# ArchieGertsman/gym-sparksched

Measured on AMD Instinct MI355X. Metric: scheduling decisions/sec (env steps/s), higher is better.
Workload: dtype f64+i32

## Files before the change

gym-sparksched_amd/csrc/decima_rollout.h:

```cpp
#pragma once
#include <type_traits>

#include "kernels.h"
#include "decima.h"
#include "decima_policy.h"

#ifndef SSIM_DR_EX_LDS
#define SSIM_DR_EX_LDS 0
#endif

struct DecimaWork {
  int64_t feat_scratch, plan, stride;
  int64_t feats, ccap, emask, depth;
  int64_t packed, total;
};
inline DecimaWork decima_work(const ssim_layout& L) {
  DecimaWork w{};
  w.feat_scratch = 0;
  w.plan = align16(decima_scratch_bytes(L.stage_cap));
  w.stride = (w.plan + decima_policy_lds_bytes(L.stage_cap, L.job_cap) + 255) & ~int64_t(255);
  int64_t o = w.stride * L.num_envs;
  w.feats = o;
  o = align16(o + (int64_t)L.num_envs * L.stage_cap * kDecimaFeatures * 4);
  w.ccap = o;
// ... 23 lines not shown
template <bool kHelp = false, bool kGreedy = false>
__device__ __forceinline__ DpAction decima_decide(
    const Params* P0, const uint8_t* obs0, const dp_f32x4* weights0, uint8_t* feat_scratch0, uint8_t* plan0,
    float* feats0, int32_t* ccap0, uint32_t* emask0, int32_t* depth0, float num_tasks_scale, float work_scale,
    uint64_t seed, uint64_t ctr, int eid, int plan_cap, uint32_t plan_lds, uint64_t* pprof, uint32_t help_lds = 0) {
  using W = WaveHip;
  const Params* P = (const Params*)(const SSIM_GLOBAL Params*)P0;
  const uint8_t* obs = (const uint8_t*)(const SSIM_GLOBAL uint8_t*)obs0;
  const dp_f32x4* weights = (const dp_f32x4*)(const SSIM_GLOBAL dp_f32x4*)weights0;
  float* feats = (float*)(SSIM_GLOBAL float*)feats0;
  int32_t* ccap = (int32_t*)(SSIM_GLOBAL int32_t*)ccap0;
  uint32_t* emask = (uint32_t*)(SSIM_GLOBAL uint32_t*)emask0;
  int32_t* depth = (int32_t*)(SSIM_GLOBAL int32_t*)depth0;
  const ssim_layout& L = P->L;
  const DecimaPolicyOut none{nullptr, nullptr, nullptr, nullptr, nullptr, nullptr, nullptr};
  const DpWGlobal wts{weights};
  DpAction act;
  DpHelp* const help = kHelp ? reinterpret_cast<DpHelp*>(g_smem + help_lds) : nullptr;
#ifdef SSIM_PROFILE
  uint64_t tp = W::clock();
#endif
#ifdef SSIM_DR_GLOBAL_ONLY
  if (false) {
#else
  if (plan_cap > 0) {
#endif
    uint8_t* pl = g_smem + plan_lds;
    DecimaView<W>{L, obs, eid}.template run<false>(num_tasks_scale, work_scale, pl, feats, ccap, emask, depth,
                                                   plan_cap);
#ifdef SSIM_PROFILE
    if (pprof != nullptr && W::lane() == 0) W::lds_add_u64(pprof - kPhDecParts + kPhDecFeat, W::clock() - tp);
#endif
    decima_policy_env<false, kHelp, kGreedy>(P, obs, feats, ccap, emask, depth, wts, plan_cap, seed, ctr, eid, pl, none, &act,
                                    pprof, kDpLdsDags, help);
  } else {
    uint8_t* fs = (uint8_t*)(SSIM_GLOBAL uint8_t*)feat_scratch0;
    uint8_t* pg = (uint8_t*)(SSIM_GLOBAL uint8_t*)plan0;
    DecimaView<W>{L, obs, eid}.template run<true>(num_tasks_scale, work_scale, fs, feats, ccap, emask, depth);
#ifdef SSIM_PROFILE
    if (pprof != nullptr && W::lane() == 0) W::lds_add_u64(pprof - kPhDecParts + kPhDecFeat, W::clock() - tp);
#endif
    decima_policy_env<true, kHelp, kGreedy>(P, obs, feats, ccap, emask, depth, wts, L.stage_cap, seed, ctr, eid, pg, none, &act,
                                   pprof, 0, help);
  }
  return act;
}

struct DecimaTimedNone {};
template <bool kTimed>
using DecimaTimedArgs = std::conditional_t<kTimed, ssim_decima_timed, DecimaTimedNone>;
template <bool kHelp = false, bool kTimed = false, bool kGreedy = false>
struct DecimaPolicy {
  static constexpr bool kTimedMode = kTimed;
  const Params* P;
  const uint8_t* obs;
  DecimaRolloutArgs a;
  DecimaTimedArgs<kTimed> t;

  template <class S>
  __device__ __forceinline__ bool in_time(const S& s) const {
    if constexpr (kTimed) return WaveHip::uni(t.clock[2 * (int64_t)s.eid]) < t.duration;
    return true;
  }
  template <class S>
  __device__ __forceinline__ bool next_episode(const S& s) const {
    if constexpr (kTimed) {
      using W = WaveHip;
      int32_t* sc = t.sched + 2 * (int64_t)s.eid;
      if (W::uni(sc[0]) < t.cap_resets) return true;
      W::sync();
      if (W::lane() == 0) sc[1] = 1;
      W::sync();
      return false;
    }
    return true;
  }
  template <class S>
  __device__ __forceinline__ void reset_episode(S& s, uint8_t* rec) const {
    if constexpr (kTimed) {
      using W = WaveHip;
      const int eid = s.eid;
      int32_t* sc = t.sched + 2 * (int64_t)eid;
      const int64_t slot = (int64_t)eid * t.cap_resets + W::uni(sc[0]);
      const uint64_t seed = W::uni(t.seeds[slot]);
      const double limit = W::uni(t.limits[slot]);
      const int last = W::uni(a.smp.cursor[(int64_t)eid * 8]) - 1;
      const int J = s.JC;
      for (int j = W::lane(); j < J; j += W::kWidth) {
        t.ep_arrival[slot * J + j] = s.jtimes(j).tarr;
        t.ep_completed[slot * J + j] = s.jtimes(j).tdone;
        t.ep_state[slot * J + j] = s.job(j).state;
      }
      W::sync();
      if (W::lane() == 0) {
        t.reset_steps[slot] = last;
        sc[0] = sc[0] + 1;
      }
      W::sync();
      s.reset_sampled(SSIM_RESET_SEED, seed, limit, rec);
    }
  }

  template <class S>
  __device__ __forceinline__ bool can_act(const S& s) const {
    using W = WaveHip;
    if (!a.autoreset && (s.h.terminated || s.frozen() || s.h.wall >= s.h.time_limit || s.h.num_jobs == 0))
// ... 261 lines not shown
```

gym-sparksched_amd/csrc/engine.h:

```cpp
#pragma once
#include <stddef.h>
#include <stdint.h>

#include "layout.h"
#include "pcg64.h"
#include "pyset.h"

#ifdef SSIM_PROFILE
#define SSIM_TIC(v) const uint64_t v = W::clock()
#define SSIM_TOC(v, ph) prof_add(ph, W::clock() - (v))
#else
#define SSIM_TIC(v) (void)0
#define SSIM_TOC(v, ph) (void)0
#endif

#ifdef SSIM_MARKERS
#define SSIM_MARK(name) asm volatile("; SSIM_MARK " name)
#else
#define SSIM_MARK(name) (void)0
#endif

#if defined(__clang__)
#pragma clang fp contract(off)
#endif

namespace ssim {

template <class W, class = void>
struct KatBadPage {
  static constexpr bool value = false;
};
template <class W>
struct KatBadPage<W, decltype((void)W::kKatBadPage)> {
  static constexpr bool value = W::kKatBadPage;
};

#if defined(__HIP_DEVICE_COMPILE__)
#define SSIM_GLOBAL __attribute__((address_space(1)))
#else
#define SSIM_GLOBAL
#endif
template <class T>
__device__ __forceinline__ T ldg(const T* p, int64_t i) {
  return ((const SSIM_GLOBAL T*)p)[i];
}

enum : int32_t { kPhPolicy = 0, kPhAction, kPhRoundCheck, kPhFulfill, kPhPop, kPhHandle, kPhPostScan, kPhObserve,
                 kPhSample, kPhPool, kPhScan, kPhLoadSave, kPhPoolBig, kPhIdleOrder, kPhDraw, kPhJobArr,
                 kPhExecArr, kPhTaskDone, kPhStageDone,
                 kPhIter,
                 kCtPoolSmall, kCtPoolBig, kCtTask, kCtIdleOrder,
                 kHist0,
                 kTEntry = kHist0 + 16, kTLoaded, kTLoopEnd, kTSaved, kTCtor, kTCopy1,
                 kPhDecFeat, kPhDecPolicy, kPhDecRecord,
                 kPhDecParts,
                 kPhReset = kPhDecParts + 10, kCtReset,
                 kCtNoEvent, kCtPredPass, kCtDeltaObs, kNumPhases };
static_assert(kNumPhases <= 64, "StateOffsets::sc_prof holds 64 sums");
#ifdef SSIM_PROFILE
#define SSIM_COUNT(ph) prof_add(ph, 1)
#else
#define SSIM_COUNT(ph) (void)0
#endif
#ifndef SSIM_POOL_STAT
#define SSIM_POOL_STAT(op, size, used) (void)0
#endif
#ifndef SSIM_FIELD_STAT
#define SSIM_FIELD_STAT(sec) (void)0
#endif
enum : int32_t { kPoolNone = -1, kPoolCommon = 0 };
enum : int32_t { kEvArrival = 1, kEvTask = 2, kEvReady = 3, kTrJobDone = 4, kTrToCommon = 5 };
enum : int32_t { kJobPending = 0, kJobActive = 1, kJobDone = 2 };
enum : int32_t { kScanAll = 0, kScanOnly = 1, kScanExcept = 2 };

struct StepIn {
  int32_t stage_idx, num_exec;
};

struct NoStop {
  static constexpr bool kCan = false;
  __device__ __forceinline__ uint64_t issue() const { return 0; }
  __device__ __forceinline__ bool hit(uint64_t) const { return false; }
};
enum : int32_t { kSimIdle = 0, kSimDecision = 1, kSimPreempted = 2 };

struct HotParams {
  const int32_t* tpl_stage_base;
  const int32_t* ts_num_tasks;
  const double* ts_rough;
  const int32_t* ts_child_base;
  const int32_t* ts_children;
  const int32_t* ts_parent_base;
  const int32_t* ts_parents;
  const int32_t* ts_fw_keymask;
  const int32_t* ts_fw_maxlevel;
  const int32_t* dur_off;
  const int32_t* dur_len;
  const double* durations;
  const uint64_t* ts_topo;
  double moving_delay, warmup_delay, beta, job_arrival_gap;
  int64_t ob_nodes, ob_edge_links, ob_dag_ptr, ob_supplies, ob_frontier, ob_sched_rank, ob_counts, ob_reward,
      ob_wall_time, ob_acc, ob_trace;
  int32_t num_templates, trace_cap, edge_cap, job_arrival_cap, topo;
  int32_t dcache;
};
static_assert(sizeof(HotParams) <= 256 && sizeof(HotParams) % 8 == 0, "one dword per lane of one VGPR");

constexpr int kIvRows = 256;
struct Params {
  HotParams hp;
  ssim_layout L;
// ... 18 lines not shown
  memset(p->iv, 0, sizeof(p->iv));
  for (int n = 0; n <= num_executors && n < kIvRows; ++n) {
    const double lo = intervals[2 * n], hi = intervals[2 * n + 1];
    if (!(lo >= 0 && lo <= 255 && hi >= 0 && hi <= 255 && lo == (double)(int)lo && hi == (double)(int)hi))
      return false;
    p->iv[n][0] = (uint8_t)lo;
    p->iv[n][1] = (uint8_t)hi;
    p->iv[n][2] = (uint8_t)exec_level_index(lo);
    p->iv[n][3] = (uint8_t)exec_level_index(hi);
  }
  return true;
}

inline void fill_hot_params(Params* p) {
  HotParams& h = p->hp;
  const ssim_dataset& D = p->D;
  h.tpl_stage_base = D.tpl_stage_base;
  h.ts_num_tasks = D.ts_num_tasks;
  h.ts_rough = D.ts_rough;
  h.ts_child_base = D.ts_child_base;
  h.ts_children = D.ts_children;
  h.ts_parent_base = D.ts_parent_base;
  h.ts_parents = D.ts_parents;
  h.ts_fw_keymask = D.ts_fw_keymask;
  h.ts_fw_maxlevel = D.ts_fw_maxlevel;
  h.dur_off = D.dur_off;
  h.dur_len = D.dur_len;
  h.durations = D.durations;
  h.ts_topo = D.ts_topo;
  h.moving_delay = p->C.moving_delay;
  h.warmup_delay = p->C.warmup_delay;
  h.beta = p->C.beta;
  h.job_arrival_gap = p->C.job_arrival_gap;
  const ssim_layout& L = p->L;
  h.ob_nodes = L.ob_nodes;
  h.ob_edge_links = L.ob_edge_links;
  h.ob_dag_ptr = L.ob_dag_ptr;
  h.ob_supplies = L.ob_supplies;
  h.ob_frontier = L.ob_frontier;
  h.ob_sched_rank = L.ob_sched_rank;
  h.ob_counts = L.ob_counts;
  h.ob_reward = L.ob_reward;
  h.ob_wall_time = L.ob_wall_time;
  h.ob_acc = L.ob_acc;
  h.ob_trace = L.ob_trace;
  h.num_templates = D.num_templates;
  h.trace_cap = L.trace_cap;
  h.edge_cap = L.edge_cap;
  h.job_arrival_cap = p->C.job_arrival_cap;
  h.topo = (p->C.max_stages <= 32 && D.ts_topo != nullptr) ? 1 : 0;
  h.dcache = 0;
}

template <class W, int kN = 0, int kJ = 0, int kS = 0>
struct Sim {
  using WT = W;
  const ssim_layout& L;
  const ssim_dataset& D;
  const ssim_config& C;
  const uint8_t (*IV)[4];
  const int32_t NE, JC, SC;
  const StateOffsets O;
  uint8_t* ghot;
  uint8_t* hot;
  uint8_t* cold;
  uint8_t* scr;
  uint8_t* obs;
  int32_t eid;
  bool res;
  bool row_lds;
  bool ex_l;
  uint8_t* xb;
  EnvHeader h;
  Pcg64 rng;
  uint32_t iv_lane;
#ifndef SSIM_EV_PAGES_GENERIC
#define SSIM_EV_PAGES_GENERIC 1
#endif
#ifndef SSIM_DUR_CACHE
#define SSIM_DUR_CACHE 1
#endif
  static constexpr int kEvPages = W::kWidth == 64 ? (kN > 0 ? (kN + 63) / 64 : SSIM_EV_PAGES_GENERIC) : 0;
  struct EvRegs {
    uint32_t tlo, thi;
    int32_t seq;
    int32_t ts;
  };
  EvRegs evr[kEvPages > 0 ? kEvPages : 1];
  __device__ __forceinline__ bool ev_in_regs() const { return kEvPages > 0 && NE <= 64 * kEvPages; }
  static constexpr bool kDurCache = W::kWidth == 64 && kN > 0 && kN <= kDurCacheMaxExecs && SSIM_DUR_CACHE;
  bool dcache_on = false;
  __device__ __forceinline__ bool dc_on() const { return kDurCache && dcache_on; }
  const HotParams* HPp;
  uint32_t hpv;
#ifdef SSIM_PROFILE
  uint64_t* prof;
  __device__ __forceinline__ void prof_add(int ph, uint64_t v) {
    if (W::lane() == 0) W::lds_add_u64(prof + ph, v);
  }
  __device__ __forceinline__ void prof_set(int ph, uint64_t v) {
    W::sync();
    if (W::lane() == 0) prof[ph] = v;
    W::sync();
  }
#endif

  __device__ __forceinline__ Sim(const Params* __restrict__ p, uint8_t* state_arena, uint8_t* lds,
                                 uint8_t* obs_arena, int32_t env_index, bool resident, bool row_cold = false,
                                 bool ex_lds = false)
// ... 221 lines not shown
    __device__ __forceinline__ UF& operator-=(int v) {
      SSIM_FIELD_STAT(kSec);
      *p = (T)(*p - v);
      return *this;
    }
  };
  template <class T>
  __device__ __forceinline__ T ld(const T* q) const {
    return W::uni(*q);
  }
  template <class T>
  __device__ __forceinline__ T ldu(const T* q, int64_t i) const {
    return W::uni(ldg(q, i));
  }

  template <class R>
  __device__ __forceinline__ R ld_rec(const R& src) const {
    static_assert(sizeof(R) % 4 == 0, "records are whole words");
    uint32_t w[sizeof(R) / 4];
    __builtin_memcpy(w, &src, sizeof(R));
    for (int i = 0; i < (int)(sizeof(R) / 4); ++i) w[i] = W::uni(w[i]);
    R r;
    __builtin_memcpy(&r, w, sizeof(R));
    return r;
  }

  __device__ __forceinline__ StageRec& stage(int g) const { return H<StageRec>(O.stages)[g]; }
  __device__ __forceinline__ JobRec& job(int j) const { return H<JobRec>(O.jobs)[j]; }
  __device__ __forceinline__ JobTimes& jtimes(int j) const { return H<JobTimes>(O.jtimes)[j]; }
  __device__ __forceinline__ ExecRec& exr(int e) const { return reinterpret_cast<ExecRec*>(xb)[e]; }
  __device__ __forceinline__ CommitRec& cm(int k) const { return H<CommitRec>(O.commits)[k]; }
  __device__ __forceinline__ PoolRec& pool(int p) const { return H<PoolRec>(O.pools)[p]; }
  __device__ __forceinline__ double* recent() const { return reinterpret_cast<double*>(cold + O.st_recent); }
  __device__ __forceinline__ UF<int16_t, 0> st_job(int g) const { return {&stage(g).job}; }
  __device__ __forceinline__ UF<int16_t, 0> st_ts(int g) const { return {&stage(g).ts}; }
  __device__ __forceinline__ UF<int16_t, 0> st_rem(int g) const { return {&stage(g).rem}; }
  __device__ __forceinline__ UF<int16_t, 0> st_exe(int g) const { return {&stage(g).exe}; }
  __device__ __forceinline__ UF<int16_t, 0> st_mov(int g) const { return {&stage(g).mov}; }
  __device__ __forceinline__ UF<int16_t, 0> st_com(int g) const { return {&stage(g).com}; }
  __device__ __forceinline__ UF<int8_t, 0> st_unmet(int g) const { return {&stage(g).unmet}; }
  __device__ __forceinline__ UF<uint8_t, 0> st_sel(int g) const { return {&stage(g).sel}; }
  __device__ __forceinline__ UF<double, 6> st_recent(int g) const { return {recent() + g}; }
  __device__ __forceinline__ bool st_completed(int g) const { return st_rem(g) == 0 && st_exe(g) == 0; }
  __device__ __forceinline__ UF<int16_t, 1> job_tpl(int j) const { return {&job(j).tpl}; }
  __device__ __forceinline__ UF<int16_t, 1> job_base(int j) const { return {&job(j).base}; }
  __device__ __forceinline__ UF<int16_t, 1> job_nst(int j) const { return {&job(j).nst}; }
  __device__ __forceinline__ UF<int16_t, 1> job_nact(int j) const { return {&job(j).nact}; }
  __device__ __forceinline__ UF<int16_t, 1> job_sat(int j) const { return {&job(j).sat}; }
  __device__ __forceinline__ UF<int16_t, 1> job_local(int j) const { return {&job(j).local}; }
  __device__ __forceinline__ UF<int16_t, 1> job_supply(int j) const { return {&job(j).supply}; }
  __device__ __forceinline__ UF<int16_t, 1> job_state(int j) const { return {&job(j).state}; }
  __device__ __forceinline__ UF<int32_t, 1> job_arr_dec(int j) const { return {&job(j).arr_dec}; }
  __device__ __forceinline__ UF<int32_t, 1> job_done_dec(int j) const { return {&job(j).done_dec}; }
  __device__ __forceinline__ UF<double, 2> job_tarr(int j) const { return {&jtimes(j).tarr}; }
  __device__ __forceinline__ UF<double, 2> job_tdone(int j) const { return {&jtimes(j).tdone}; }
  __device__ __forceinline__ UF<int16_t, 3> ex_loc(int e) const { return {&exr(e).loc}; }
  __device__ __forceinline__ UF<int16_t, 3> ex_job(int e) const { return {&exr(e).job}; }
  __device__ __forceinline__ UF<int16_t, 3> ex_task(int e) const { return {&exr(e).task}; }
  __device__ __forceinline__ UF<int16_t, 3> ex_busy(int e) const { return {&exr(e).busy}; }
  __device__ __forceinline__ UF<double, 4> ev_t(int e) const { return {&exr(e).ev_t}; }
  __device__ __forceinline__ UF<int32_t, 4> ev_seq(int e) const { return {&exr(e).ev_seq}; }
  __device__ __forceinline__ UF<int16_t, 4> ev_type(int e) const { return {&exr(e).ev_type}; }
  __device__ __forceinline__ UF<int16_t, 4> ev_stage(int e) const { return {&exr(e).ev_stage}; }
  __device__ __forceinline__ int32_t job_pool(int j) const { return 1 + j; }
  __device__ __forceinline__ int32_t stage_pool(int g) const { return 1 + JC + g; }
  __device__ __forceinline__ bool is_stage_pool(int p) const { return p > JC; }
  __device__ __forceinline__ int32_t pool_stage(int p) const { return p - 1 - JC; }
  __device__ __forceinline__ int32_t pool_job(int p) const {
    if (p <= 0) return -1;
    if (p <= JC) return p - 1;
    return st_job(p - 1 - JC);
  }
  __device__ __forceinline__ PySetMeta* pmeta(int p) const { return reinterpret_cast<PySetMeta*>(&pool(p)); }
  __device__ __forceinline__ uint8_t* ptab(int p) const { return cold + O.pool_tab + (int64_t)p * tab_stride_for(NE); }
  __device__ __forceinline__ UF<int16_t, 5> cfrom(int p) const { return {&pool(p).cfrom}; }
  __device__ __forceinline__ int pool_size(int p) const { return p < 0 ? 0 : (int)W::uni(pool(p).used); }

  __device__ __forceinline__ int32_t source_job() const {
    return (h.source <= kPoolCommon) ? -1 : pool_job(h.source);
  }
  __device__ __forceinline__ int committable() {
    if (h.source < 0) return 0;
    SSIM_FIELD_STAT(10);
    const PoolRec pr = pool(h.source);
    const int n = (int)W::uni(pr.used) - (int)W::uni(pr.cfrom);
    check(n >= 0);
    return n;
  }
  __device__ __forceinline__ int demand(int g) const { return st_rem(g) - (st_mov(g) + st_com(g)); }

  __device__ __forceinline__ void supply_add(int job, int n) {
    if (job < 0)
      h.supply_none += n;
    else
      job_supply(job) += n;
  }

  __device__ __forceinline__ void add_commitment(int n, int dst) {
    const int src = h.source;
    check(src >= 0);
    if (src < 0) return;
    int hit = -1, freeslot = -1;
    SSIM_FIELD_STAT(13);
    const int hw = h.commit_hw;
    for (int k0 = 0; k0 < commit_cap_for(NE); k0 += W::kWidth) {
      if (k0 >= hw) break;
// ... 1177 lines not shown
      release_idle_one(src, e);
      return;
    }
    goto_stage(e, pool_stage(dst));
  }

  __device__ __forceinline__ void fulfill_from_source() {
    int32_t* idle = S<int32_t>(O.sc_keys_a);
    int32_t* plan = S<int32_t>(O.sc_plan);
    const int n_idle = idle_order(h.source, idle);
    const int n_plan = h.source >= 0 ? commit_plan(h.source, plan) : 0;
    int k = 0;
    for (int c = 0; c < n_plan; ++c) {
      const int dst = ld(plan + 2 * c);
      int n = ld(plan + 2 * c + 1);
      check(dst >= 0 && n > 0);
      while (n > 0 && k < n_idle && !frozen()) {
        const int e = ld(idle + k++);
        fulfill(e, dst);
        n--;
      }
    }
    check(k == n_idle);
  }

  __device__ __forceinline__ void commit_leftovers() {
    const int n = committable();
    if (n > 0) add_commitment(n, kPoolCommon);
  }

  __device__ __forceinline__ bool release(int e, int g, bool changed) {
    const int dst = peek_commitment(stage_pool(g));
    if (dst != kPoolNone) {
      fulfill(e, dst);
      return true;
    }
    ex_task(e) = -1;
    if (changed) release_idle_one(stage_pool(g), e);
    return false;
  }

  __device__ __forceinline__ void on_job_arrival(int j) {
    job_state(j) = kJobActive;
    job_arr_dec(j) = h.decisions;
    int16_t* aj = H<int16_t>(O.active_jobs);
    int16_t* as = H<int16_t>(O.active_stages);
    if (W::lane() == 0) aj[h.n_active_jobs] = (int16_t)j;
    const int base = job_base(j), n = job_nst(j), tsb = ldu(HP(tpl_stage_base), (int)job_tpl(j));
    const int32_t* const nt = HP(ts_num_tasks);
    const int32_t* const pb = HP(ts_parent_base);
    const int32_t* const fwk = HP(ts_fw_keymask);
    const int32_t* const fwm = HP(ts_fw_maxlevel);
    const double* const rough = HP(ts_rough);
    for (int k0 = 0; k0 <= n; k0 += W::kWidth) {
      const int k = k0 + W::lane();
      if (k <= n) {
        const int p = (k == n) ? job_pool(j) : stage_pool(base + k);
        ps_init(pmeta(p), pool(p).tab);
        cfrom(p) = 0;
        if (k < n) {
          const int g = base + k, ts = tsb + k;
          StageRec r;
          r.job = (int16_t)j;
          r.ts = (int16_t)ts;
          r.rem = (int16_t)ldg(nt, ts);
          r.exe = 0;
          r.mov = 0;
          r.com = 0;
          r.unmet = (int8_t)(ldg(pb, ts + 1) - ldg(pb, ts));
          r.sel = 0;
          r.fw_keymask = (uint8_t)ldg(fwk, ts);
          r.fw_maxlevel = (uint8_t)ldg(fwm, ts);
          stage(g) = r;
          recent()[g] = ldg(rough, ts);
          as[h.n_active_stages + k] = (int16_t)g;
        }
      }
    }
    W::sync();
    h.n_active_jobs += 1;
    h.n_active_stages += n;
    if (pool_size(kPoolCommon) > 0) h.source = kPoolCommon;
  }

  __device__ __forceinline__ void on_executor_arrival(int e, int g) {
    SSIM_FIELD_STAT(11);
    const StageRec sraw = stage(g);
    const ExecRec xraw = exr(e);
    const StageRec sr = ld_rec(sraw);
    const int j = sr.job;
    check(W::uni(xraw.task) < 0);
    job_local(j) += 1;
    ex_job(e) = (int16_t)j;
    st_mov(g) = (int16_t)(sr.mov - 1);
    check(sr.mov - 1 >= 0);
    move_to_pool(e, job_pool(j), false);
    goto_stage(e, g);
  }

  __device__ __forceinline__ bool stage_completed(int j, int g) {
    check(st_unmet(g) == 0);
    list_remove(H<int16_t>(O.active_stages), h.n_active_stages, g);
    h.n_active_stages -= 1;
    job_nact(j) -= 1;
    const int ts = st_ts(g), base = job_base(j);
    bool changed = false;
    if (topo_masks()) {
      uint32_t cm = (uint32_t)(ldu(HP(ts_topo), ts) >> 32);
      while (cm) {
        const int c = base + __builtin_ctz(cm);
        cm &= cm - 1;
        st_unmet(c) -= 1;
        if (st_unmet(c) == 0 && !st_completed(c)) changed = true;
      }
      return changed;
    }
    const int kb = ldu(HP(ts_child_base), ts), ke = ldu(HP(ts_child_base), ts + 1);
    for (int k = kb; k < ke; ++k) {
      const int c = base + ldu(HP(ts_children), k);
      st_unmet(c) -= 1;
      if (st_unmet(c) == 0 && !st_completed(c)) changed = true;
    }
    return changed;
  }

  __device__ __forceinline__ void job_completed(int j) {
    if (pool_size(job_pool(j)) > 0) release_idle_all(job_pool(j));
    check(pool_size(job_pool(j)) == 0);
    list_remove(H<int16_t>(O.active_jobs), h.n_active_jobs, j);
    h.n_active_jobs -= 1;
    h.n_completed += 1;
    job_state(j) = kJobDone;
    job_tdone(j) = h.wall;
    job_done_dec(j) = h.decisions;
    trace(h.wall, kTrJobDone, -1, j, -1, -1);
  }

  __device__ __forceinline__ void on_task_done(int e, int g, StageRec s, ExecRec x, const DurDesc& dd) {
    SSIM_MARK("task_done_begin");
    const int j = s.job;
    check(!(s.rem == 0 && s.exe == 0));
    s.exe = (int16_t)(s.exe - 1);
    x.busy = 0;
    if (s.rem > 0) {
      run_next_task_rec(e, g, s, x, dd);
      stage(g) = s;
      exr(e) = x;
      SSIM_MARK("task_done_fast_end");
      return;
    }
    stage(g) = s;
    exr(e) = x;
    SSIM_TIC(t_sd);
    bool changed = false;
    if (st_completed(g)) changed = stage_completed(j, g);
    SSIM_TOC(t_sd, kPhStageDone);
    if (job_nact(j) == 0) job_completed(j);
    const bool had = release(e, g, changed);
    if (changed)
      h.source = job_pool(j);
    else if (!had)
      h.source = stage_pool(g);
  }

  __device__ __forceinline__ bool pop_event(double* t, int* kind, int* e, int* g, int* seq) {
    constexpr int kSpan = W::kWidth < 16 ? W::kWidth : (kN > 0 && kN <= 16) ? 16 : 64;
    double bt = 0.0;
    int bseq = 0x7FFFFFFF, be = -1, btype = 0, bstage = -1;
    const bool have_arr = h.arrivals < h.num_jobs;
    const double ta_lane = have_arr ? jtimes(h.arrivals).tarr : 0.0;
// ... 120 lines not shown
      if (committable() == 0) {
        SSIM_TOC(t_s, kPhPostScan);
        continue;
      }
      const bool found = scan_sched(source_job());
      if (!found) {
        release_idle_all(kPoolNone);
        h.source = kPoolNone;
      }
      SSIM_TOC(t_s, kPhPostScan);
      if (found) return kSimDecision;
    }
  }

  __device__ __forceinline__ double jobtime(double t0, int dec) {
    const double span = h.wall - t0;
    if (span == 0.0) return 0.0;
    double part = 0.0;
    const double beta = HP(beta);
    for (int j0 = 0; j0 < h.arrivals; j0 += W::kWidth) {
      const int j = j0 + W::lane();
      if (j < h.arrivals) {
        const JobRec jr = job(j);
        const JobTimes jt = jtimes(j);
        const int st = jr.state;
        const bool in_union = st == kJobActive || (st == kJobDone && jr.done_dec == dec && jr.arr_dec < dec);
        if (in_union) {
          const double ta = jt.tarr;
          const double a = ta > t0 ? ta : t0;
          const double tc = st == kJobDone ? jt.tdone : h.wall;
          const double b = tc < h.wall ? tc : h.wall;
          if (beta == 0.0)
            part += b - a;
          else
            part += exp(-beta * 1e-3 * (a - t0)) - exp(-beta * 1e-3 * (b - t0));
        }
      }
    }
    double total = W::sum_d(part);
    if (beta > 0.0) total /= beta;
    return total;
  }

#ifndef SSIM_NT_OBS
#define SSIM_NT_OBS 0
#endif
  template <class T>
  __device__ __forceinline__ static void obs_st(T* p, T v) {
    if constexpr (SSIM_NT_OBS && W::kWidth == 64)
      W::st_nt(p, v);
    else
      *p = v;
  }
  __device__ __forceinline__ void observe(double reward, bool step_done = false, int ncommit = -1,
                                          bool delta = false) {
    const bool dl = SSIM_TAIL_DELTA && delta && obs_live;
    const bool masks = SSIM_TAIL_MASKS && pred_ok;
    pred_ok = false;
    const uint64_t pm0 = pred_m0, pm1 = pred_m1, pm2 = pred_m2;
    if (!masks) SSIM_COUNT(kCtPredPass);
    if (dl) SSIM_COUNT(kCtDeltaObs);
    const int n = h.n_active_stages;
    const int src_job = source_job();
    const int16_t* act = H<int16_t>(O.active_stages);
    int16_t* sched = H<int16_t>(O.sched_list);
    int16_t* row_of = row_lds ? S<int16_t>(O.sc_row_of) : reinterpret_cast<int16_t*>(cold + O.row_of);
    float* nodes = reinterpret_cast<float*>(obs + HP(ob_nodes)) + (int64_t)eid * SC * 3;
    uint8_t* front = obs + HP(ob_frontier) + (int64_t)eid * SC;
    int32_t* srank = reinterpret_cast<int32_t*>(obs + HP(ob_sched_rank)) + (int64_t)eid * SC;
    const TopoView tv = topo_view();
    const int ecap = HP(edge_cap);
    const int16_t* ajl = H<int16_t>(O.active_jobs);
    for (int k0 = 0; k0 < h.n_active_jobs; k0 += W::kWidth) {
      const int k = k0 + W::lane();
      if (k < h.n_active_jobs) job(ajl[k]).pick = 0x7FFFFFFF;
    }
    W::sync();
    int nsched = 0;
    for (int i0 = 0; i0 < n; i0 += W::kWidth) {
      const int i = i0 + W::lane();
      const bool ok = i < n;
      const int g = ok ? act[i] : -1;
      bool s;
      if (masks) {
        const uint64_t pm = i0 < 64 ? pm0 : i0 < 128 ? pm1 : pm2;
        s = ok && ((pm >> (i & 63)) & 1) != 0;
      } else {
        s = ok && stage_pred(g, kScanAll, -1, src_job, tv);
      }
      const uint64_t m = W::ballot(s);
      const int r = nsched + W::rank(m);
      if (ok) {
        StageRec sr{};
        if (!dl || s) sr = stage(g);
        if (!dl) {
          obs_st(nodes + 3 * i + 0, (float)sr.rem);
          obs_st(nodes + 3 * i + 1, (float)recent()[g]);
          obs_st(front + i, (uint8_t)(sr.unmet == 0 ? 1 : 0));
          row_of[g] = (int16_t)i;
        }
        obs_st(nodes + 3 * i + 2, s ? 1.0f : 0.0f);
        obs_st(srank + i, s ? r : -1);
        if (s) {
          sched[r] = (int16_t)g;
          W::amin(&job(sr.job).pick, (sr.unmet == 0 ? 0 : 0x10000) | r);
        }
      }
      nsched += W::popc(m);
    }
    W::sync();
    const int nj = h.n_active_jobs;
    const int16_t* aj = H<int16_t>(O.active_jobs);
    int32_t* ptr = reinterpret_cast<int32_t*>(obs + HP(ob_dag_ptr)) + (int64_t)eid * (JC + 1);
    int32_t* sup = reinterpret_cast<int32_t*>(obs + HP(ob_supplies)) + (int64_t)eid * JC;
    int src_idx = nj, run = 0;
    for (int k0 = 0; k0 < nj; k0 += W::kWidth) {
      const int k = k0 + W::lane();
      const bool ok = k < nj;
      const int j = ok ? aj[k] : -1;
      const JobRec jr = ok ? job(j) : JobRec{};
      if (!dl) {
        const int cnt = ok ? jr.nact : 0;
        int total = 0;
        const int ex = W::excl_scan(cnt, &total);
        if (ok) obs_st(ptr + k, run + ex);
        run += total;
      }
      if (ok) obs_st(sup + k, (int32_t)jr.supply);
      const uint64_t ms = W::ballot(ok && j == src_job);
      if (ms) src_idx = k0 + W::ffs(ms);
    }
    if (!dl) {
      if (W::lane() == 0) obs_st(ptr + nj, run);
      check(run == n);
    }
    int64_t* links = reinterpret_cast<int64_t*>(obs + HP(ob_edge_links)) + (int64_t)eid * ecap * 2;
    int ne = dl ? obs_ne : 0;
    for (int i0 = 0; !dl && i0 < n; i0 += W::kWidth) {
      const int i = i0 + W::lane();
      const bool ok = i < n;
      const int g = ok ? act[i] : -1;
      int cnt = 0, cb = 0, ce = 0, base = 0;
      uint32_t live = 0;
      if (ok) {
        const StageRec sr = stage(g);
        base = job(sr.job).base;
        if (tv.bits) {
          uint32_t cm = (uint32_t)(ldg(tv.ts_topo, sr.ts) >> 32);
          while (cm) {
            const int b = __builtin_ctz(cm);
            cm &= cm - 1;
            const StageRec c = stage(base + b);
            if (!(c.rem == 0 && c.exe == 0)) live |= 1u << b;
          }
          cnt = __builtin_popcount(live);
        } else {
          cb = ldg(tv.child_base, sr.ts);
          ce = ldg(tv.child_base, sr.ts + 1);
          for (int k = cb; k < ce; ++k) {
            const StageRec c = stage(base + ldg(tv.children, k));
            if (!(c.rem == 0 && c.exe == 0)) cnt++;
          }
        }
      }
      int total = 0;
      const int ex = W::excl_scan(cnt, &total);
      if (ok) {
        int o = ne + ex;
        if (tv.bits) {
          while (live && o < ecap) {
            const int c = base + __builtin_ctz(live);
            live &= live - 1;
            obs_st(links + 2 * o + 0, (int64_t)i);
            obs_st(links + 2 * o + 1, (int64_t)row_of[c]);
            o++;
          }
        } else {
          for (int k = cb; k < ce; ++k) {
            const int c = base + ldg(tv.children, k);
            const StageRec cr = stage(c);
            if (!(cr.rem == 0 && cr.exe == 0) && o < ecap) {
              obs_st(links + 2 * o + 0, (int64_t)i);
              obs_st(links + 2 * o + 1, (int64_t)row_of[c]);
              o++;
            }
          }
        }
      }
      ne += total;
    }
    if (ne > ecap) fail(SSIM_ERR_CAPACITY);
    obs_live = true;
    obs_ne = ne;
    h.n_sched = nsched;
    h.src_idx = src_idx;
    h.stage_idx_n = n + 1;
    EnvAcc a = ld_rec(*H<EnvAcc>(O.acc));
    a.nodes += n;
    a.edges += ne;
    a.jobs += nj;
    a.events += h.step_events;
    if (step_done) a.decisions += 1;
    *H<EnvAcc>(O.acc) = a;
    int64_t* const acc = reinterpret_cast<int64_t*>(obs + HP(ob_acc)) + (int64_t)eid * kNumAcc;
    int32_t* const cnts = reinterpret_cast<int32_t*>(obs + HP(ob_counts)) + (int64_t)eid * SSIM_NUM_COUNTS;
    double* const rew = reinterpret_cast<double*>(obs + HP(ob_reward)) + eid;
    double* const wall = reinterpret_cast<double*>(obs + HP(ob_wall_time)) + eid;
    if (ncommit < 0) ncommit = committable();
    W::sync();
    if (W::lane() == 0) {
      acc[0] = a.nodes;
      acc[1] = a.edges;
      acc[2] = a.jobs;
      acc[3] = a.events;
      acc[4] = a.decisions;
      acc[5] = a.episodes;
      acc[6] = 0;
      acc[7] = 0;
      cnts[SSIM_OC_NUM_NODES] = n;
      cnts[SSIM_OC_NUM_EDGES] = ne;
      cnts[SSIM_OC_NUM_JOBS] = nj;
      cnts[SSIM_OC_COMMITTABLE] = ncommit;
      cnts[SSIM_OC_SOURCE_JOB_IDX] = src_idx;
      cnts[SSIM_OC_NUM_SCHEDULABLE] = nsched;
      cnts[SSIM_OC_TERMINATED] = h.terminated;
      cnts[SSIM_OC_TRUNCATED] = h.wall >= h.time_limit ? 1 : 0;
      cnts[SSIM_OC_ERR] = (int32_t)h.err;
      cnts[SSIM_OC_DECISIONS] = h.decisions;
      cnts[SSIM_OC_EVENTS] = h.events;
      cnts[SSIM_OC_NUM_COMPLETED] = h.n_completed;
      cnts[SSIM_OC_NUM_ARRIVED] = h.arrivals;
      cnts[SSIM_OC_TRACE_LEN] = h.trace_len;
      cnts[SSIM_OC_STEP_EVENTS] = h.step_events;
      cnts[SSIM_OC_EPISODE] = h.episode;
      *rew = reward;
      *wall = h.wall;
    }
    W::sync();
  }

  __device__ __forceinline__ void write_err_only(uint32_t transient) {
    int32_t* const cnts = reinterpret_cast<int32_t*>(obs + HP(ob_counts)) + (int64_t)eid * SSIM_NUM_COUNTS;
    W::sync();
// ... 296 lines not shown
```

gym-sparksched_amd/csrc/kernels.h:

```cpp
#pragma once
#include <hip/hip_runtime.h>

#include "sparksched.h"
#include "engine.h"
#include "policy.h"
#include "rollout.h"
#include "wave_hip.h"

using namespace ssim;

extern __shared__ __attribute__((aligned(16))) uint8_t g_smem[];

__device__ __forceinline__ bool env_idle(const Params* __restrict__ P, const uint8_t* state, int eid) {
  const EnvHeader* gh =
      reinterpret_cast<const EnvHeader*>(state + kParamsReserve + (int64_t)eid * P->L.env_bytes + P->O.hdr);
  return gh->terminated || (gh->err & SSIM_ERR_STICKY) || gh->num_jobs == 0;
}

#ifndef SSIM_HBM_ROLLOUT_WAVES
#define SSIM_HBM_ROLLOUT_WAVES 4
#endif
#ifndef SSIM_HBM_STEP_WAVES
#define SSIM_HBM_STEP_WAVES 4
#endif
// ... 27 lines not shown
  }
  __device__ __forceinline__ bool hit(uint64_t v) const { return on && WaveHip::uni(v) != 0; }
};

template <bool kRes, int kN, int kJ, int kS>
__global__ __attribute__((amdgpu_flat_work_group_size(1, 64), amdgpu_waves_per_eu(kRes ? 1 : SSIM_HBM_STEP_WAVES))) void k_step(const Params* __restrict__ P, uint8_t* state, uint8_t* obs,
                                             const int32_t* __restrict__ stage_idx,
                                             const int32_t* __restrict__ num_exec) {
  const int eid = blockIdx.x;
  if (env_idle(P, state, eid)) return;
  Sim<WaveHip, kN, kJ, kS> s(P, state, g_smem, obs, eid, kRes, false, !kRes);
  StepIn a;
  a.stage_idx = stage_idx[eid];
  a.num_exec = num_exec[eid];
  s.load_hot();
  s.load_header();
  if (s.pending()) {
    s.resume(NoStop());
    s.write_err_only(SSIM_ERR_PENDING);
  } else {
    s.step_loaded(a);
  }
  s.save_hot();
}

template <bool kRes, int kN, int kJ, int kS, class Pol>
__device__ __forceinline__ void rollout_body(const Params* __restrict__ P, uint8_t* state, uint8_t* obs,
                                                const Pol& pol, int num_steps, int flags,
                                                const double* __restrict__ limits, uint8_t* reset,
                                                int32_t* action_log, uint64_t* prof_out, int64_t budget,
                                                const int32_t* __restrict__ env_steps, bool row_cold = false,
                                                bool ex_lds = true) {
  const int eid = blockIdx.x;
  const int B = P->L.num_envs;
  if (budget > 0 && eid == 0 && WaveHip::lane() <= kStopLines)
    *reinterpret_cast<unsigned long long*>(state + kTicketOffset + ((flags & kFlagTicketSlot) ? 0 : kTicketSlotBytes) +
                                           kTicketStride * WaveHip::lane()) = 0ull;
  if (env_steps != nullptr) {
    const int n = env_steps[eid];
    num_steps = n < num_steps ? n : num_steps;
    if (num_steps <= 0) return;
  }
  const bool autoreset = (flags & SSIM_ROLLOUT_AUTORESET) != 0;
  if (!autoreset && !Pol::kTimedMode && action_log == nullptr && env_idle(P, state, eid)) return;
  const int slot = (flags & kFlagTicketSlot) ? 1 : 0;
  const TicketStop stop{budget > 0 ? state + kTicketOffset + kTicketSlotBytes * slot : nullptr, budget,
                        eid % kStopLines, budget > 0 && (flags & SSIM_ROLLOUT_PREEMPT) != 0};
  RolloutCursor c{0, 0, 0};
  const double limit = limits != nullptr ? limits[eid] : __builtin_inf();
  uint8_t* rec = reset + (int64_t)eid * P->L.reset_stride;
#ifdef SSIM_PROFILE
  const uint64_t rt_entry = WaveHip::realtime();
#endif
  Sim<WaveHip, kN, kJ, kS> s(P, state, g_smem, obs, eid, kRes, row_cold, ex_lds && !kRes);
#ifdef SSIM_PROFILE
  s.prof_set(kTCtor, WaveHip::realtime());
#endif
  s.load_hot();
#ifdef SSIM_PROFILE
  s.prof_set(kTEntry, rt_entry);
  s.prof_set(kTLoaded, WaveHip::realtime());
#endif
  const auto reset_in_place = [&](Sim<WaveHip, kN, kJ, kS>& x) {
    if constexpr (Pol::kTimedMode)
      pol.reset_episode(x, rec);
    else
      x.reset_sampled(SSIM_RESET_CONTINUE, 0ull, limit, rec);
  };
  rollout_loop(s, pol, stop, c, B, eid, num_steps, autoreset, action_log, reset_in_place);
  if (c.granted > 0) stop.give_back(c.granted);
#ifdef SSIM_PROFILE
  s.prof_set(kTLoopEnd, WaveHip::realtime());
#endif
  s.save_hot();
#ifdef SSIM_PROFILE
  s.prof_set(kTSaved, WaveHip::realtime());
  WaveHip::sync();
  if (prof_out != nullptr)
    for (int p = WaveHip::lane(); p < kNumPhases; p += 64) prof_out[(int64_t)eid * kNumPhases + p] = s.prof[p];
#else
  (void)prof_out;
#endif
}

#define SSIM_ROLLOUT_ARGS                                                                                       \
  const Params *__restrict__ P, uint8_t *state, uint8_t *obs, int kind, uint64_t seed, int num_steps, int flags, \
      const double *__restrict__ limits, uint8_t *reset, int32_t *action_log, uint64_t *prof_out, int64_t budget, \
      const int32_t *__restrict__ env_steps
#define SSIM_ROLLOUT_WAVES(kRes) ((kRes) ? 1 : SSIM_HBM_ROLLOUT_WAVES)
template <bool kRes, int kN, int kJ, int kS>
__global__ __attribute__((amdgpu_flat_work_group_size(1, 64), amdgpu_waves_per_eu(SSIM_ROLLOUT_WAVES(kRes)))) void k_rollout(SSIM_ROLLOUT_ARGS) {
  rollout_body<kRes, kN, kJ, kS, HeuristicPolicy>(P, state, obs, HeuristicPolicy{kind, seed}, num_steps, flags, limits,
                                                  reset, action_log, prof_out, budget, env_steps);
}
template <bool kRes, int kN, int kJ, int kS>
__global__ __attribute__((amdgpu_flat_work_group_size(1, 64), amdgpu_waves_per_eu(SSIM_ROLLOUT_WAVES(kRes)))) void k_rollout_warmup(SSIM_ROLLOUT_ARGS) {
  rollout_body<kRes, kN, kJ, kS, HeuristicPolicy>(P, state, obs, HeuristicPolicy{kind, seed}, num_steps, flags, limits,
                                                  reset, action_log, prof_out, budget, env_steps);
}
template <bool kRes>
__global__ __attribute__((amdgpu_flat_work_group_size(1, 64), amdgpu_waves_per_eu(SSIM_ROLLOUT_WAVES(kRes)))) void k_rollout_prio(SSIM_ROLLOUT_ARGS) {
  (void)seed;
  rollout_body<kRes, 0, 0, 0, PrioPolicy>(P, state, obs, PrioPolicy{kind}, num_steps, flags, limits, reset, action_log,
                                          prof_out, budget, env_steps);
}

template <class WV, bool kRes, int kN, int kJ, int kS, int kTag>
__global__ __attribute__((amdgpu_flat_work_group_size(1, 64), amdgpu_waves_per_eu(SSIM_ROLLOUT_WAVES(kRes)))) void k_set_trace(const Params* __restrict__ P, uint8_t* state, uint8_t* obs,
                                                  const int32_t* __restrict__ ops, int n_ops, int width,
                                                  int32_t* orders) {
  Sim<WV, kN, kJ, kS> s(P, state, g_smem, obs, 0, kRes);
  if constexpr (kRes) s.load_hot();
  const int p = s.job_pool(0);
  ps_init(s.pmeta(p), s.pool(p).tab);
  int32_t* out = s.template S<int32_t>(s.O.sc_keys_a);
  for (int k = 0; k < n_ops; ++k) {
// ... 50 lines not shown
```

gym-sparksched_amd/csrc/layout.h:

```cpp
#pragma once
#include <stdint.h>
#include <string.h>

#include "sparksched.h"

namespace ssim {

struct EnvHeader {
  double wall;
  double time_limit;
  uint64_t rng_s_hi, rng_s_lo, rng_i_hi, rng_i_lo;
  uint32_t rng_has32, rng_u32;
  int32_t num_jobs;
  int32_t arrivals;
  int32_t seq;
  int32_t n_active_jobs;
  int32_t n_active_stages;
  int32_t n_completed;
  int32_t source;
  int32_t commit_seq;
  int32_t supply_none;
  int32_t n_sched;
  int32_t n_selected;
  int32_t decisions;
  int32_t events;
  int32_t terminated;
  uint32_t err;
  int32_t stage_idx_n;
  int32_t episode;
  int32_t trace_len;
  int32_t step_events;
  int32_t src_idx;
  int32_t err_line;
  int32_t commit_hw;
};
static_assert(sizeof(EnvHeader) % 16 == 0, "header must keep 16-B alignment");

struct EnvAcc {
  int64_t nodes, edges, jobs, events, decisions, episodes;
  double pend_t0;
  int64_t pending;
};
static_assert(sizeof(EnvAcc) % 16 == 0, "accumulator record");

struct StageRec {
  int16_t job, ts;
  int16_t rem, exe;
  int16_t mov, com;
  int8_t unmet;
  uint8_t sel;
  uint8_t fw_keymask;
  uint8_t fw_maxlevel;
};
static_assert(sizeof(StageRec) == 16, "stage record");

struct JobRec {
  int16_t tpl, base, nst, nact;
  int16_t sat, local, supply, state;
  int32_t arr_dec, done_dec;
  int32_t pick;
  int32_t pad;
};
static_assert(sizeof(JobRec) == 32, "job record");

struct JobTimes {
  double tarr, tdone;
};

struct ExecRec {
  int16_t loc, job, task, busy;
  int16_t ev_type, ev_stage;
  int32_t ev_seq;
  double ev_t;
  int64_t pad;
};
static_assert(sizeof(ExecRec) == 32, "executor record");

struct CommitRec {
  int16_t src, dst, cnt, pad;
  int32_t ord, pad2;
};
static_assert(sizeof(CommitRec) == 16, "commitment record");

struct PoolRec {
  uint16_t mask, fill, used;
  int16_t cfrom;
  uint8_t tab[8];
};
static_assert(sizeof(PoolRec) == 16, "pool record");

constexpr int kNumLevels = 8;
constexpr int kNumAcc = 8;
constexpr int kTraceBytes = 32;
constexpr int64_t kResetHeadBytes = 64;
static_assert(sizeof(ssim_reset_record) <= kResetHeadBytes, "reset record");
constexpr int64_t kLdsBudget = 64 * 1024;
constexpr int64_t kLdsPerCu = 160 * 1024;
constexpr int64_t kHbmWorkgroupsPerCu = 16;
constexpr int64_t kLdsBudgetBig = 160 * 1024;
constexpr int64_t kBigLdsMaxEnvs = 256;
constexpr int64_t kChipCus = 256;
constexpr int64_t lds_concurrent_envs(int64_t need, int64_t chip_cus = kChipCus) {
  const int64_t per_cu = kLdsPerCu / (need > 0 ? need : 1);
  return chip_cus * (per_cu < 4 ? per_cu : 4);
}

struct TraceRec {
  double t;
  int32_t kind;
  int32_t exec;
  int32_t job;
  int32_t stage;
  int32_t seq;
  int32_t pad;
// ... 36 lines not shown
  O.jobs = o;
  o = align16(o + (int64_t)sizeof(JobRec) * J);
  O.jtimes = o;
  o = align16(o + (int64_t)sizeof(JobTimes) * J);
  O.active_jobs = o;
  o = align16(o + 2 * J);
  O.execs = o;
  o = align16(o + (int64_t)sizeof(ExecRec) * N);
  O.sel_list = o;
  o = align16(o + 2 * (N + 1));
  O.commits = o;
  o = align16(o + (int64_t)sizeof(CommitRec) * C);
  O.stages = o;
  o = align16(o + (int64_t)sizeof(StageRec) * S);
  O.pools = o;
  o = align16(o + (int64_t)sizeof(PoolRec) * P);
  O.active_stages = o;
  o = align16(o + 2 * S);
  O.sched_list = o;
  o = align16(o + 2 * S);
  O.hot_bytes = o;

  int64_t c = 0;
  O.st_recent = c;
  c = align16(c + 8 * S);
  O.pool_tab = c;
  c = align16(c + TS * P);
  O.row_of = c;
  c = align16(c + 2 * S);
  O.cold_bytes = c;
  O.env_bytes = O.hot_bytes + O.cold_bytes;

  int64_t s = 0;
  O.sc_execs = s;
  s = align16(s + (int64_t)sizeof(ExecRec) * N);
  O.sc_keys_a = s;
  s = align16(s + 4 * (N + 1));
  O.sc_keys_b = s;
  s = align16(s + 4 * (N + 1));
  O.sc_plan = s;
  s = align16(s + 8 * C);
  O.sc_tab_a = s;
  s = align16(s + T);
  O.sc_tab_b = s;
  s = align16(s + T);
  O.sc_tab_p = s;
  s = align16(s + T);
  O.sc_dcache = s;
  s = align16(s + (N <= kDurCacheMaxExecs ? 4 * 24 * N : 0));
  O.sc_bits = s;
  s = align16(s + (T > 64 && T <= kPagedTabMax ? 16 : 0));
  O.sc_prof = s;
#ifdef SSIM_PROFILE
  s += 8 * 64;
#endif
  O.scratch_hbm_bytes = align16(s);
  O.sc_row_of = O.scratch_hbm_bytes;
  s = align16(O.sc_row_of + 2 * S);
  O.scratch_bytes = s;
  return O;
}

inline bool compute_layout(const ssim_config& cfg, ssim_layout* L, StateOffsets* O, int64_t chip_cus = kChipCus) {
  if (cfg.num_envs <= 0 || cfg.num_executors <= 0 || cfg.num_executors > 250 || cfg.job_cap <= 0 ||
      cfg.max_stages <= 0 || cfg.max_stages > 128  || cfg.max_edges < 0 ||
      cfg.trace_cap < 0)
    return false;
  memset(L, 0, sizeof(*L));
  const int64_t B = cfg.num_envs, N = cfg.num_executors, J = cfg.job_cap;
  const int64_t S = J * cfg.max_stages, E = J * (cfg.max_edges > 0 ? cfg.max_edges : 1);
  const int64_t P = 1 + J + S, T = set_cap_for((int)N), C = commit_cap_for((int)N);
  if (P >= 32767) return false;
  L->num_envs = (int32_t)B;
  L->num_executors = (int32_t)N;
  L->job_cap = (int32_t)J;
  L->stage_cap = (int32_t)S;
  L->edge_cap = (int32_t)E;
  L->pool_cap = (int32_t)P;
  L->set_cap = (int32_t)T;
  L->commit_cap = (int32_t)C;
  L->trace_cap = cfg.trace_cap;

  *O = state_offsets(N, J, S);
  L->env_bytes = O->env_bytes;
  L->state_bytes = 4096 + L->env_bytes * B;
  L->scratch_bytes = O->scratch_bytes;
  const int64_t need = O->hot_bytes + O->scratch_bytes;
  O->lds_resident = (!(cfg.flags & SSIM_CFG_FORCE_HBM) &&
                     ((need <= kLdsBudget && 2 * B <= 3 * lds_concurrent_envs(need, chip_cus)) ||
                      (need <= kLdsBudgetBig && B <= kBigLdsMaxEnvs)))
                        ? 1 : 0;
  L->lds_resident = O->lds_resident;
  O->row_of_lds = (O->lds_resident || O->scratch_bytes * kHbmWorkgroupsPerCu <= kLdsPerCu) ? 1 : 0;
  O->lds_bytes = O->lds_resident ? O->hot_bytes + O->scratch_bytes
                                 : O->row_of_lds ? O->scratch_bytes : O->scratch_hbm_bytes;
  L->lds_bytes = O->lds_bytes;
  if (O->lds_resident) {
    const int64_t per_cu = lds_concurrent_envs(need, chip_cus) / (chip_cus > 0 ? chip_cus : 1);
    O->lds_share = B <= chip_cus ? kLdsBudgetBig : kLdsPerCu / (per_cu > 1 ? per_cu : 1);
  } else {
    O->lds_share = kLdsPerCu / kHbmWorkgroupsPerCu;
  }
  L->lds_share = O->lds_share;
  L->chip_cus = chip_cus;

  int64_t b = 0;
  auto otake = [&](int64_t bytes) {
// ... 24 lines not shown
```

gym-sparksched_amd/csrc/rollout.h:

```cpp
#pragma once
#include "engine.h"
#include "policy.h"

namespace ssim {

struct NoBudget : NoStop {
  uint8_t* base = nullptr;
  bool on = false;
  __device__ __forceinline__ int64_t claim(int64_t, int64_t&) const { return 0; }
  __device__ __forceinline__ void give_back(int64_t) const {}
};

struct HeuristicPolicy {
  static constexpr bool kTimedMode = false;
  int kind;
  uint64_t seed;
  template <class S>
  __device__ __forceinline__ bool can_act(const S&) const {
    return true;
  }
  template <class S>
  __device__ __forceinline__ bool act(S& s, int , StepIn* a) const {
    *a = sim_policy_legacy(s, kind, seed);
    return true;
  }
  template <class S>
  __device__ __forceinline__ void done(S&) const {}
  template <class S>
  __device__ __forceinline__ void rejected(S&) const {}
};

struct PrioPolicy {
  static constexpr bool kTimedMode = false;
  int kind;
  template <class S>
  __device__ __forceinline__ bool can_act(const S&) const {
    return true;
  }
  template <class S>
  __device__ __forceinline__ bool act(S& s, int , StepIn* a) const {
    *a = sim_policy_prio(s, kind);
    return true;
  }
  template <class S>
  __device__ __forceinline__ void done(S&) const {}
  template <class S>
  __device__ __forceinline__ void rejected(S&) const {}
};

struct RolloutCursor {
  int k;
  int64_t granted;
  int64_t last;
};
template <class SimT, class Pol, class StopT, class ResetFn>
__device__ __forceinline__ void rollout_loop(SimT& s, const Pol& pol, const StopT& stop, RolloutCursor& c, int B,
                                            int eid, int num_steps, bool autoreset, int32_t* action_log,
                                            const ResetFn& reset_env) {
  using W = typename SimT::WT;
  for (;;) {
#ifdef SSIM_PROFILE
    const uint64_t t0 = W::clock();
#endif
    s.load_header();
    if constexpr (Pol::kTimedMode) {
      if (s.h.num_jobs > 0 && !s.frozen() && (s.h.terminated || s.h.wall >= s.h.time_limit) && !s.pending()) {
        if (!pol.next_episode(s)) break;
        reset_env(s);
        continue;
      }
      if (!s.pending() && !pol.in_time(s)) break;
    }
    if (autoreset && s.h.num_jobs > 0 && !s.frozen() && (s.h.terminated || s.h.wall >= s.h.time_limit) &&
        !s.pending()) {
      if (stop.on && c.granted == 0 && (c.granted = stop.claim(B, c.last)) == 0) break;
#ifdef SSIM_PROFILE
      const uint64_t tr = W::clock();
#endif
      reset_env(s);
#ifdef SSIM_PROFILE
      s.prof_add(kPhReset, W::clock() - tr);
      s.prof_add(kCtReset, 1);
#endif
      continue;
    }
    double st0 = 0.0;
    bool simulate;
    if (s.pending()) {
      st0 = s.take_pending();
      simulate = true;
    } else {
      if (c.k >= num_steps) break;
      if (!pol.can_act(s)) break;
      if (stop.base != nullptr) {
        if (!autoreset && (s.h.terminated || s.frozen())) break;
        if (c.granted == 0 && (c.granted = stop.claim(B, c.last)) == 0) break;
        --c.granted;
      }
      StepIn a;
      if (!pol.act(s, c.k, &a)) break;
#ifdef SSIM_PROFILE
      s.prof_add(kPhPolicy, W::clock() - t0);
#endif
      if (action_log != nullptr && W::lane() == 0) {
        action_log[((int64_t)c.k * B + eid) * 2 + 0] = a.stage_idx;
        action_log[((int64_t)c.k * B + eid) * 2 + 1] = a.num_exec;
      }
      ++c.k;
      W::sync();
      simulate = s.step_begin(a, &st0);
      if (!simulate && s.rejected) {
        pol.rejected(s);
        s.fail(SSIM_ERR_INVARIANT);
        s.store_header();
        s.write_err_only(0u);
        break;
      }
      if (!simulate) pol.done(s);
    }
    if (simulate) {
      if (!s.finish_step(st0, stop)) break;
      pol.done(s);
    }
#ifdef SSIM_PROFILE
    {
      const uint64_t dc = W::clock() - t0;
      int b = 63 - __builtin_clzll(dc | 1ull) - 10;
      b = b < 0 ? 0 : b > 15 ? 15 : b;
      s.prof_add(kHist0 + b, 1);
      s.prof_add(kPhIter, dc);
    }
#endif
  }
}

}
```

Measured before the change: 36.06 million.

## Defer observation row writes for heuristic policies until rollout end

For heuristic and priority policies, the per-step observe now computes only the decision state (schedulable set, picks, source index) and marks the observation rows stale. The full node, frontier, pointer, supply and edge-link rows are written once when the rollout loop exits. Each job now tracks its remaining edge count so the total number of edges can be carried without rebuilding the link table every step. The cost removed is the per-step row and edge materialisation; in exchange the code is more complex, and any consumer that reads obs rows between steps could see stale data.

```diff
diff --git a/gym-sparksched_amd/csrc/decima_rollout.h b/gym-sparksched_amd/csrc/decima_rollout.h
--- a/gym-sparksched_amd/csrc/decima_rollout.h
+++ b/gym-sparksched_amd/csrc/decima_rollout.h
@@ -99,6 +99,7 @@
 template <bool kHelp = false, bool kTimed = false, bool kGreedy = false>
 struct DecimaPolicy {
   static constexpr bool kTimedMode = kTimed;
+  static constexpr bool kLazyRows = false;
   const Params* P;
   const uint8_t* obs;
   DecimaRolloutArgs a;
diff --git a/gym-sparksched_amd/csrc/engine.h b/gym-sparksched_amd/csrc/engine.h
--- a/gym-sparksched_amd/csrc/engine.h
+++ b/gym-sparksched_amd/csrc/engine.h
@@ -55,8 +55,8 @@
                  kPhDecFeat, kPhDecPolicy, kPhDecRecord,
                  kPhDecParts,
                  kPhReset = kPhDecParts + 10, kCtReset,
-                 kCtNoEvent, kCtPredPass, kCtDeltaObs, kNumPhases };
-static_assert(kNumPhases <= 64, "StateOffsets::sc_prof holds 64 sums");
+                 kCtNoEvent, kCtPredPass, kCtDeltaObs, kCtLazyObs, kCtRowFlush, kNumPhases };
+static_assert(kNumPhases <= 72, "StateOffsets::sc_prof holds 72 sums");
 #ifdef SSIM_PROFILE
 #define SSIM_COUNT(ph) prof_add(ph, 1)
 #else
@@ -181,9 +181,10 @@
   h.dcache = 0;
 }
 
-template <class W, int kN = 0, int kJ = 0, int kS = 0>
+template <class W, int kN = 0, int kJ = 0, int kS = 0, bool kLazy = false>
 struct Sim {
   using WT = W;
+  static constexpr bool kLazyObs = kLazy;
   const ssim_layout& L;
   const ssim_dataset& D;
   const ssim_config& C;
@@ -511,6 +512,7 @@
   __device__ __forceinline__ UF<int16_t, 1> job_state(int j) const { return {&job(j).state}; }
   __device__ __forceinline__ UF<int32_t, 1> job_arr_dec(int j) const { return {&job(j).arr_dec}; }
   __device__ __forceinline__ UF<int32_t, 1> job_done_dec(int j) const { return {&job(j).done_dec}; }
+  __device__ __forceinline__ UF<int32_t, 1> job_edges(int j) const { return {&job(j).edges}; }
   __device__ __forceinline__ UF<double, 2> job_tarr(int j) const { return {&jtimes(j).tarr}; }
   __device__ __forceinline__ UF<double, 2> job_tdone(int j) const { return {&jtimes(j).tdone}; }
   __device__ __forceinline__ UF<int16_t, 3> ex_loc(int e) const { return {&exr(e).loc}; }
@@ -1794,6 +1796,9 @@
     const int32_t* const fwk = HP(ts_fw_keymask);
     const int32_t* const fwm = HP(ts_fw_maxlevel);
     const double* const rough = HP(ts_rough);
+    const bool bits = topo_masks();
+    const uint64_t* const topo = bits ? HP(ts_topo) : nullptr;
+    int ec = 0;
     for (int k0 = 0; k0 <= n; k0 += W::kWidth) {
       const int k = k0 + W::lane();
       if (k <= n) {
@@ -1816,9 +1821,16 @@
           stage(g) = r;
           recent()[g] = ldg(rough, ts);
           as[h.n_active_stages + k] = (int16_t)g;
+          if (bits) ec += __builtin_popcount((uint32_t)(ldg(topo, ts) >> 32));
         }
       }
     }
+    int etot = 0;
+    if (bits)
+      W::excl_scan(ec, &etot);
+    else
+      etot = ldu(HP(ts_child_base), tsb + n) - ldu(HP(ts_child_base), tsb);
+    job_edges(j) = etot;
     W::sync();
     h.n_active_jobs += 1;
     h.n_active_stages += n;
@@ -1849,6 +1861,7 @@
     bool changed = false;
     if (topo_masks()) {
       uint32_t cm = (uint32_t)(ldu(HP(ts_topo), ts) >> 32);
+      job_edges(j) -= __builtin_popcount(cm);
       while (cm) {
         const int c = base + __builtin_ctz(cm);
         cm &= cm - 1;
@@ -1858,6 +1871,7 @@
       return changed;
     }
     const int kb = ldu(HP(ts_child_base), ts), ke = ldu(HP(ts_child_base), ts + 1);
+    job_edges(j) -= ke - kb;
     for (int k = kb; k < ke; ++k) {
       const int c = base + ldu(HP(ts_children), k);
       st_unmet(c) -= 1;
@@ -2084,11 +2098,39 @@
     else
       *p = v;
   }
+#if defined(SSIM_PROFILE) || !defined(__HIP_DEVICE_COMPILE__)
+  static constexpr bool kCheckEdges = true;
+#else
+  static constexpr bool kCheckEdges = false;
+#endif
+  bool rows_stale = false;
   __device__ __forceinline__ void observe(double reward, bool step_done = false, int ncommit = -1,
                                           bool delta = false) {
-    const bool dl = SSIM_TAIL_DELTA && delta && obs_live;
-    const bool masks = SSIM_TAIL_MASKS && pred_ok;
-    pred_ok = false;
+    if constexpr (kLazyObs) {
+      SSIM_COUNT(kCtLazyObs);
+      observe_parts<true, false>(reward, step_done, ncommit, delta);
+      rows_stale = true;
+    } else {
+      observe_parts<true, true>(reward, step_done, ncommit, delta);
+    }
+  }
+  __device__ __forceinline__ void flush_rows() {
+    if (!rows_stale || frozen() || pending()) return;
+    SSIM_TIC(t_o);
+    SSIM_COUNT(kCtRowFlush);
+    observe_parts<false, true>(0.0, false, -1, false);
+    SSIM_TOC(t_o, kPhObserve);
+    rows_stale = false;
+    if (kCheckEdges && frozen()) {
+      store_header();
+      write_err_only(0u);
+    }
+  }
+  template <bool kDec, bool kRows>
+  __device__ __forceinline__ void observe_parts(double reward, bool step_done, int ncommit, bool delta) {
+    const bool dl = kDec && SSIM_TAIL_DELTA && delta && obs_live;
+    const bool masks = kDec && SSIM_TAIL_MASKS && pred_ok;
+    if (kDec) pred_ok = false;
     const uint64_t pm0 = pred_m0, pm1 = pred_m1, pm2 = pred_m2;
     if (!masks) SSIM_COUNT(kCtPredPass);
     if (dl) SSIM_COUNT(kCtDeltaObs);
@@ -2103,11 +2145,11 @@
     const TopoView tv = topo_view();
     const int ecap = HP(edge_cap);
     const int16_t* ajl = H<int16_t>(O.active_jobs);
-    for (int k0 = 0; k0 < h.n_active_jobs; k0 += W::kWidth) {
+    for (int k0 = 0; kDec && k0 < h.n_active_jobs; k0 += W::kWidth) {
       const int k = k0 + W::lane();
       if (k < h.n_active_jobs) job(ajl[k]).pick = 0x7FFFFFFF;
     }
-    W::sync();
+    if (kDec) W::sync();
     int nsched = 0;
     for (int i0 = 0; i0 < n; i0 += W::kWidth) {
       const int i = i0 + W::lane();
@@ -2124,16 +2166,18 @@
       const int r = nsched + W::rank(m);
       if (ok) {
         StageRec sr{};
-        if (!dl || s) sr = stage(g);
-        if (!dl) {
+        if ((kRows && !dl) || (kDec && s)) sr = stage(g);
+        if (kRows && !dl) {
           obs_st(nodes + 3 * i + 0, (float)sr.rem);
           obs_st(nodes + 3 * i + 1, (float)recent()[g]);
           obs_st(front + i, (uint8_t)(sr.unmet == 0 ? 1 : 0));
           row_of[g] = (int16_t)i;
         }
-        obs_st(nodes + 3 * i + 2, s ? 1.0f : 0.0f);
-        obs_st(srank + i, s ? r : -1);
-        if (s) {
+        if (kRows) {
+          obs_st(nodes + 3 * i + 2, s ? 1.0f : 0.0f);
+          obs_st(srank + i, s ? r : -1);
+        }
+        if (kDec && s) {
           sched[r] = (int16_t)g;
           W::amin(&job(sr.job).pick, (sr.unmet == 0 ? 0 : 0x10000) | r);
         }
@@ -2146,29 +2190,37 @@
     int32_t* ptr = reinterpret_cast<int32_t*>(obs + HP(ob_dag_ptr)) + (int64_t)eid * (JC + 1);
     int32_t* sup = reinterpret_cast<int32_t*>(obs + HP(ob_supplies)) + (int64_t)eid * JC;
     int src_idx = nj, run = 0;
+    int ne_carried = 0;
     for (int k0 = 0; k0 < nj; k0 += W::kWidth) {
       const int k = k0 + W::lane();
       const bool ok = k < nj;
       const int j = ok ? aj[k] : -1;
       const JobRec jr = ok ? job(j) : JobRec{};
-      if (!dl) {
+      if (kRows && !dl) {
         const int cnt = ok ? jr.nact : 0;
         int total = 0;
         const int ex = W::excl_scan(cnt, &total);
         if (ok) obs_st(ptr + k, run + ex);
         run += total;
       }
-      if (ok) obs_st(sup + k, (int32_t)jr.supply);
-      const uint64_t ms = W::ballot(ok && j == src_job);
-      if (ms) src_idx = k0 + W::ffs(ms);
-    }
-    if (!dl) {
+      if ((!kRows || kCheckEdges) && !dl) {
+        int total = 0;
+        W::excl_scan(ok ? (int)jr.edges : 0, &total);
+        ne_carried += total;
+      }
+      if (kRows && ok) obs_st(sup + k, (int32_t)jr.supply);
+      if (kDec) {
+        const uint64_t ms = W::ballot(ok && j == src_job);
+        if (ms) src_idx = k0 + W::ffs(ms);
+      }
+    }
+    if (kRows && !dl) {
       if (W::lane() == 0) obs_st(ptr + nj, run);
       check(run == n);
     }
     int64_t* links = reinterpret_cast<int64_t*>(obs + HP(ob_edge_links)) + (int64_t)eid * ecap * 2;
-    int ne = dl ? obs_ne : 0;
-    for (int i0 = 0; !dl && i0 < n; i0 += W::kWidth) {
+    int ne = dl ? obs_ne : kRows ? 0 : ne_carried;
+    for (int i0 = 0; kRows && !dl && i0 < n; i0 += W::kWidth) {
       const int i = i0 + W::lane();
       const bool ok = i < n;
       const int g = ok ? act[i] : -1;
@@ -2221,6 +2273,11 @@
       }
       ne += total;
     }
+    if constexpr (kRows && kCheckEdges) {
+      if (!dl) check(ne == (kDec ? ne_carried : obs_ne));
+      if (!kDec) check(ne == ne_carried);
+    }
+    if constexpr (!kDec) return;
     if (ne > ecap) fail(SSIM_ERR_CAPACITY);
     obs_live = true;
     obs_ne = ne;
diff --git a/gym-sparksched_amd/csrc/kernels.h b/gym-sparksched_amd/csrc/kernels.h
--- a/gym-sparksched_amd/csrc/kernels.h
+++ b/gym-sparksched_amd/csrc/kernels.h
@@ -103,7 +103,8 @@
 #ifdef SSIM_PROFILE
   const uint64_t rt_entry = WaveHip::realtime();
 #endif
-  Sim<WaveHip, kN, kJ, kS> s(P, state, g_smem, obs, eid, kRes, row_cold, ex_lds && !kRes);
+  using SimT = Sim<WaveHip, kN, kJ, kS, Pol::kLazyRows>;
+  SimT s(P, state, g_smem, obs, eid, kRes, row_cold, ex_lds && !kRes);
 #ifdef SSIM_PROFILE
   s.prof_set(kTCtor, WaveHip::realtime());
 #endif
@@ -112,7 +113,7 @@
   s.prof_set(kTEntry, rt_entry);
   s.prof_set(kTLoaded, WaveHip::realtime());
 #endif
-  const auto reset_in_place = [&](Sim<WaveHip, kN, kJ, kS>& x) {
+  const auto reset_in_place = [&](SimT& x) {
     if constexpr (Pol::kTimedMode)
       pol.reset_episode(x, rec);
     else
diff --git a/gym-sparksched_amd/csrc/layout.h b/gym-sparksched_amd/csrc/layout.h
--- a/gym-sparksched_amd/csrc/layout.h
+++ b/gym-sparksched_amd/csrc/layout.h
@@ -59,7 +59,7 @@
   int16_t sat, local, supply, state;
   int32_t arr_dec, done_dec;
   int32_t pick;
-  int32_t pad;
+  int32_t edges;
 };
 static_assert(sizeof(JobRec) == 32, "job record");
 
@@ -202,7 +202,7 @@
   s = align16(s + (T > 64 && T <= kPagedTabMax ? 16 : 0));
   O.sc_prof = s;
 #ifdef SSIM_PROFILE
-  s += 8 * 64;
+  s += 8 * 72;
 #endif
   O.scratch_hbm_bytes = align16(s);
   O.sc_row_of = O.scratch_hbm_bytes;
diff --git a/gym-sparksched_amd/csrc/rollout.h b/gym-sparksched_amd/csrc/rollout.h
--- a/gym-sparksched_amd/csrc/rollout.h
+++ b/gym-sparksched_amd/csrc/rollout.h
@@ -13,6 +13,7 @@
 
 struct HeuristicPolicy {
   static constexpr bool kTimedMode = false;
+  static constexpr bool kLazyRows = true;
   int kind;
   uint64_t seed;
   template <class S>
@@ -32,6 +33,7 @@
 
 struct PrioPolicy {
   static constexpr bool kTimedMode = false;
+  static constexpr bool kLazyRows = true;
   int kind;
   template <class S>
   __device__ __forceinline__ bool can_act(const S&) const {
@@ -132,6 +134,7 @@
     }
 #endif
   }
+  if constexpr (SimT::kLazyObs) s.flush_rows();
 }
 
 }
```

New measurement: 37.68 million (median of 6 runs). 4.5% higher.
